# OmerMersin/video-stab

Measured on AMD Instinct MI355X. Metric: stabilized frames/sec @1080p (whole job; warp-stage HBM GB/s in roofline), higher is better.
Workload: dtype u8

## Files before the change

video-stab_amd/csrc/k_gftt.hip:

```cpp
#include <cstdio>
#include <cstdlib>

#include <cstring>

#include "vs_common.h"

namespace vsd {
namespace {

constexpr int TW = 64, TH = 16, NT = 256;
constexpr int MAX_BS = 7;

constexpr int SORT_CAP = 8192;
constexpr int CELLS_MAX = 2560;
constexpr int SLOTS = 4;
constexpr int ACC_MAX = 4096;
constexpr int SEL_NT = 256;
constexpr int NMS_ROWS = 8;

__device__ __forceinline__ uint32_t order_key(float v) {
    uint32_t b = __float_as_uint(v);
    return (b & 0x80000000u) ? ~b : (b | 0x80000000u);
}
__device__ __forceinline__ float key_to_float(uint32_t k) {
    uint32_t b = (k & 0x80000000u) ? (k & 0x7FFFFFFFu) : ~k;
    return __uint_as_float(b);
}

template <int BS>
__device__ __forceinline__ void min_eigen_tile(const uint8_t* __restrict__ gray, size_t stride, int w,
                                               int h, int bs_arg, float f1, float* __restrict__ eig,
                                               uint32_t* __restrict__ max_key) {
    constexpr int BSM = BS ? BS : MAX_BS;
    __shared__ uint8_t g[TH + BSM - 1 + 2][TW + BSM - 1 + 2 + 2];
    __shared__ float cxx[TH + BSM - 1][TW + BSM - 1 + 1], cxy[TH + BSM - 1][TW + BSM - 1 + 1], cyy[TH + BSM - 1][TW + BSM - 1 + 1];
    __shared__ uint32_t smax[NT / 64];
    const int bs = BS ? BS : bs_arg;
    const int tid = threadIdx.x;
    const int x0 = blockIdx.x * TW, y0 = blockIdx.y * TH;
    const int anchor = bs / 2, hi = bs - 1 - anchor;
    const int gx0 = x0 - anchor - 1, gy0 = y0 - anchor - 1;
    const int GW = TW + bs - 1 + 2, GH = TH + bs - 1 + 2;
    const int CW = TW + bs - 1, CH = TH + bs - 1;
    const float f0 = 2.f * f1;
    const bool interior = gx0 >= 0 && gy0 >= 0 && gx0 + GW <= w && gy0 + GH <= h;
    if (interior) {
        constexpr int NG = ((TW + BSM - 1 + 2) * (TH + BSM - 1 + 2) + NT - 1) / NT;
        const uint8_t* gb = gray + ((size_t)gy0 * stride + gx0);
        uint8_t v[NG];
        int ly[NG], lx[NG];
#pragma unroll
        for (int k = 0; k < NG; k++) {
            const int i = tid + NT * k;
            ly[k] = i / GW; lx[k] = i - ly[k] * GW;
            v[k] = i < GW * GH ? gb[(size_t)ly[k] * stride + lx[k]] : (uint8_t)0;
        }
#pragma unroll
        for (int k = 0; k < NG; k++)
            if (tid + NT * k < GW * GH) g[ly[k]][lx[k]] = v[k];
    } else {
        for (int i = tid; i < GW * GH; i += NT) {
            const int ly = i / GW, lx = i - ly * GW;
            g[ly][lx] = gray[(size_t)reflect101(gy0 + ly, h) * stride + reflect101(gx0 + lx, w)];
        }
    }
    __syncthreads();
    for (int i = tid; i < CW * CH; i += NT) {
        const int cy = i / CW, cx = i - cy * CW;
        const int px = x0 - anchor + cx, py = y0 - anchor + cy;
        float vxx = 0.f, vxy = 0.f, vyy = 0.f;
        if (interior || (px >= -anchor && px <= w - 1 + hi && py >= -anchor && py <= h - 1 + hi)) {
            const int qx = (interior ? px : reflect101(px, w)) - gx0, qy = (interior ? py : reflect101(py, h)) - gy0;
            const int a00 = g[qy - 1][qx - 1], a01 = g[qy - 1][qx], a02 = g[qy - 1][qx + 1];
            const int a10 = g[qy][qx - 1], a11 = g[qy][qx], a12 = g[qy][qx + 1];
            const int a20 = g[qy + 1][qx - 1], a21 = g[qy + 1][qx], a22 = g[qy + 1][qx + 1];
            const float r0 = (float)(a02 - a00), r1 = (float)(a12 - a10), r2 = (float)(a22 - a20);
            const float dx = (r0 + r2) * f1 + r1 * f0;
            const float t0 = (float)a01 * f0 + (float)(a00 + a02) * f1;
            const float t2 = (float)a21 * f0 + (float)(a20 + a22) * f1;
            const float dy = t2 - t0;
            (void)a11;
            vxx = dx * dx; vxy = dx * dy; vyy = dy * dy;
        }
        cxx[cy][cx] = vxx; cxy[cy][cx] = vxy; cyy[cy][cx] = vyy;
    }
    __syncthreads();
    uint32_t kmax = 0;
    for (int i = tid; i < TW * TH; i += NT) {
        const int ty = i / TW, tx = i - ty * TW;
        const int x = x0 + tx, y = y0 + ty;
        if (x < w && y < h) {
            double s0 = 0, s1 = 0, s2 = 0;
            for (int j = 0; j < bs; j++) {
                double r0 = 0, r1 = 0, r2 = 0;
                for (int k = 0; k < bs; k++) {
                    r0 += (double)cxx[ty + j][tx + k];
                    r1 += (double)cxy[ty + j][tx + k];
                    r2 += (double)cyy[ty + j][tx + k];
                }
                s0 += r0; s1 += r1; s2 += r2;
            }
            const float a = (float)s0 * 0.5f, b = (float)s1, c = (float)s2 * 0.5f;
            const float d = (a - c) * (a - c) + b * b;
            const float e = (a + c) - sqrtf(d);
            eig[(size_t)y * w + x] = e;
            const uint32_t k = order_key(e);
            kmax = k > kmax ? k : kmax;
        }
    }
#pragma unroll
    for (int off = 32; off >= 1; off >>= 1) {
        const uint32_t o = __shfl_xor(kmax, off, 64);
        kmax = o > kmax ? o : kmax;
    }
    if ((tid & 63) == 0) smax[tid >> 6] = kmax;
    __syncthreads();
    if (tid == 0) {
        uint32_t m = smax[0];
        for (int i = 1; i < NT / 64; i++) m = smax[i] > m ? smax[i] : m;
        atomicMax(max_key, m);
    }
}

template <int BS>
__global__ __launch_bounds__(NT) void min_eigen_kernel(const uint8_t* __restrict__ gray, size_t stride, int w,
                                                       int h, int bs, float f1, float* __restrict__ eig,
                                                       uint32_t* __restrict__ max_key) {
    min_eigen_tile<BS>(gray, stride, w, h, bs, f1, eig, max_key);
}

__device__ __forceinline__ void nms_row(const float* __restrict__ eig, int w, int h, double quality,
                                        const uint32_t* __restrict__ max_key,
                                        unsigned long long* __restrict__ cand, int cap,
                                        int32_t* __restrict__ counters) {
    const int x = blockIdx.x * blockDim.x + threadIdx.x;
    const float maxv = key_to_float(*max_key);
    const float thr = (float)((double)maxv * quality);
    const int lane = threadIdx.x & 63;
    float centre[NMS_ROWS];
    {
        const int xc = min(max(x, 0), w - 1);
#pragma unroll
        for (int k = 0; k < NMS_ROWS; k++) centre[k] = eig[(size_t)min((int)blockIdx.y * NMS_ROWS + k, h - 1) * w + xc];
    }
#pragma unroll
    for (int k = 0; k < NMS_ROWS; k++) {
    const int y = blockIdx.y * NMS_ROWS + k;
    if (y >= h) break;
    bool is_cand = false;
    float v = 0.f;
    if (x >= 1 && x < w - 1 && y >= 1 && y < h - 1) {
        const float* r = eig + (size_t)y * w + x;
        v = centre[k] > thr ? centre[k] : 0.f;
        if (v != 0.f) {
            float m = v;
#pragma unroll
            for (int j = -1; j <= 1; j++)
#pragma unroll
                for (int i = -1; i <= 1; i++) {
                    const float n = r[j * w + i];
                    const float tn = n > thr ? n : 0.f;
                    m = tn > m ? tn : m;
                }
            is_cand = v == m;
        }
    }
    const unsigned long long mask = __ballot(is_cand);
    if (!mask) continue;
    int base = 0;
    if (lane == __ffsll((long long)mask) - 1) base = atomicAdd(&counters[0], __popcll(mask));
    base = __builtin_amdgcn_readlane(base, __ffsll((long long)mask) - 1);
    if (!is_cand) continue;
    const int pos = base + __popcll(mask & ((1ull << lane) - 1ull));
    if (pos < cap) cand[pos] = ((unsigned long long)order_key(v) << 32) | (uint32_t)(y * w + x);
    else counters[2] = 1;
    }
}

__global__ __launch_bounds__(NT) void nms_kernel(const float* __restrict__ eig, int w, int h, double quality,
                                                 const uint32_t* __restrict__ max_key,
                                                 unsigned long long* __restrict__ cand, int cap,
                                                 int32_t* __restrict__ counters) {
    nms_row(eig, w, h, quality, max_key, cand, cap, counters);
}

struct SelArgs {
    const unsigned long long* cand;
    int32_t* counters;
    int cap, w, h, max_corners;
    int min_dist2_i;
    int use_dist;
    int cell, gw, gh;
    float* out_pts;
    int32_t* out_count;
};

template <int E>
__device__ __forceinline__ void bitonic_sort_desc(unsigned long long* keys, int tid) {
    unsigned long long v[E];
#pragma unroll
    for (int r = 0; r < E; r++) v[r] = keys[tid + SEL_NT * r];
    const int n = SEL_NT * E;
    for (int k = 2; k <= n; k <<= 1) {
        for (int j = k >> 1; j > 0; j >>= 1) {
            if (j < 64) {
#pragma unroll
                for (int r = 0; r < E; r++) {
                    const int i = tid + SEL_NT * r;
                    const unsigned int lo = (unsigned int)__shfl_xor((int)(unsigned int)v[r], j, 64);
                    const unsigned int hi = (unsigned int)__shfl_xor((int)(unsigned int)(v[r] >> 32), j, 64);
                    const unsigned long long o = ((unsigned long long)hi << 32) | lo;
                    const bool keep_max = ((i & k) == 0) == ((i & j) == 0);
                    v[r] = keep_max ? (v[r] > o ? v[r] : o) : (v[r] < o ? v[r] : o);
                }
            } else {
                __syncthreads();
#pragma unroll
                for (int r = 0; r < E; r++) keys[tid + SEL_NT * r] = v[r];
                __syncthreads();
#pragma unroll
                for (int r = 0; r < E; r++) {
                    const int i = tid + SEL_NT * r;
                    const unsigned long long o = keys[i ^ j];
                    const bool keep_max = ((i & k) == 0) == ((i & j) == 0);
                    v[r] = keep_max ? (v[r] > o ? v[r] : o) : (v[r] < o ? v[r] : o);
                }
            }
        }
    }
    __syncthreads();
#pragma unroll
    for (int r = 0; r < E; r++) keys[tid + SEL_NT * r] = v[r];
    __syncthreads();
}

__device__ __forceinline__ void select_corners(const SelArgs& a) {
    __shared__ unsigned long long keys[SORT_CAP];
    __shared__ uint32_t cell_cnt[CELLS_MAX];
    __shared__ uint32_t cell_pts[CELLS_MAX * SLOTS];
    __shared__ uint32_t acc_xy[ACC_MAX];
    __shared__ int s_m, s_nacc, s_done, s_cnt, s_overflow;
    __shared__ unsigned long long s_upper;
    const int tid = threadIdx.x;
    int ncand = a.counters[0];
    if (ncand > a.cap) ncand = a.cap;
    const int ncells = a.gw * a.gh;
    const bool grid_ok = a.use_dist && ncells <= CELLS_MAX;
    if (grid_ok) for (int i = tid; i < ncells; i += SEL_NT) cell_cnt[i] = 0;
    if (tid == 0) { s_nacc = 0; s_done = 0; s_upper = ~0ull; s_overflow = 0; }
    __syncthreads();

    int want = 1400;
    while (true) {
        const unsigned long long upper = s_upper;
        __syncthreads();
        if (tid == 0) s_cnt = 0;
        __syncthreads();
        int remaining;
        if (upper == ~0ull) {
            remaining = ncand;
        } else {
            int local = 0;
            for (int i = tid; i < ncand; i += SEL_NT) local += a.cand[i] < upper ? 1 : 0;
            if (local) atomicAdd(&s_cnt, local);
            __syncthreads();
            remaining = s_cnt;
        }
        if (remaining == 0) break;
        unsigned long long lo = 0;
        if (remaining > want + want / 2) {
            uint32_t* hist = reinterpret_cast<uint32_t*>(keys);
            unsigned long long prefix = 0;
            int above = 0;
            for (int shift = 56; shift >= 0; shift -= 8) {
                __syncthreads();
                hist[tid] = 0;
                __syncthreads();
                for (int i = tid; i < ncand; i += SEL_NT) {
                    const unsigned long long k = a.cand[i];
                    if (k < upper && (shift == 56 || (k >> (shift + 8)) == (prefix >> (shift + 8)))) atomicAdd(&hist[(uint32_t)(k >> shift) & 255u], 1u);
                }
                __syncthreads();
                if (tid == 0) {
                    int acc = above, bsel = 0;
                    for (int v = 255; v >= 0; v--) {
                        if (acc + (int)hist[v] >= want) { bsel = v; break; }
                        acc += (int)hist[v];
                    }
                    s_m = bsel;
                    s_cnt = acc;
                }
                __syncthreads();
                const int bsel = s_m, over = s_cnt, inbin = (int)hist[bsel];
                prefix |= (unsigned long long)bsel << shift;
                if (over + inbin <= SORT_CAP) { lo = prefix; break; }
                above = over;
                lo = prefix;
            }
        }
        __syncthreads();
        if (tid == 0) s_m = 0;
        __syncthreads();
        for (int i = tid; i < ncand; i += SEL_NT) {
            const unsigned long long k = a.cand[i];
            if (k >= lo && k < upper) {
                const int p = atomicAdd(&s_m, 1);
                if (p < SORT_CAP) keys[p] = k;
            }
        }
        __syncthreads();
        const int m = s_m < SORT_CAP ? s_m : SORT_CAP;
        int np2 = SEL_NT;
        while (np2 < m) np2 <<= 1;
        for (int i = m + tid; i < np2; i += SEL_NT) keys[i] = 0ull;
        __syncthreads();
        switch (np2 / SEL_NT) {
            case 1: bitonic_sort_desc<1>(keys, tid); break;
            case 2: bitonic_sort_desc<2>(keys, tid); break;
            case 4: bitonic_sort_desc<4>(keys, tid); break;
            case 8: bitonic_sort_desc<8>(keys, tid); break;
            case 16: bitonic_sort_desc<16>(keys, tid); break;
            default: bitonic_sort_desc<32>(keys, tid); break;
        }
        const unsigned long long last_key = m > 0 ? keys[m - 1] : 0ull;
        __syncthreads();
        for (int i = tid; i < m; i += SEL_NT) {
            const int idx = (int)(uint32_t)keys[i];
            const int y = idx / a.w, x = idx - y * a.w;
            const int xc = x / a.cell, yc = y / a.cell;
            keys[i] = (unsigned long long)((uint32_t)x | ((uint32_t)y << 16)) |
                      ((unsigned long long)((uint32_t)xc | ((uint32_t)yc << 16)) << 32);
        }
        __syncthreads();
        if (tid < 64) {
            const int lane = tid;
            int nacc = s_nacc;
            volatile uint32_t* vcnt = cell_cnt;
            volatile uint32_t* vpts = cell_pts;
            volatile uint32_t* vacc = acc_xy;
            const int md2 = a.min_dist2_i;
            bool full = false;
            for (int base = 0; base < m && !full; base += 64) {
                const int i = base + lane;
                const bool has = i < m;
                const unsigned long long e = has ? keys[i] : 0ull;
                const uint32_t xy = (uint32_t)e;
                const int x = (int)(xy & 0xFFFFu), y = (int)(xy >> 16);
                const int xc = (int)((uint32_t)(e >> 32) & 0xFFFFu), yc = (int)((uint32_t)(e >> 48));
                bool ok = has;
                if (a.use_dist && ok) {
                    if (grid_ok) {
                        int cidx[9];
                        uint32_t cnt[9];
#pragma unroll
                        for (int q = 0; q < 9; q++) {
                            const int cx = xc + (q % 3) - 1, cy = yc + (q / 3) - 1;
                            const bool in = cx >= 0 && cx < a.gw && cy >= 0 && cy < a.gh;
                            cidx[q] = in ? cy * a.gw + cx : -1;
                        }
#pragma unroll
                        for (int q = 0; q < 9; q++) cnt[q] = cidx[q] >= 0 ? vcnt[cidx[q]] : 0u;
#pragma unroll
                        for (int q = 0; q < 9; q++) {
                            const int c = cnt[q] < (uint32_t)SLOTS ? (int)cnt[q] : SLOTS;
                            for (int sl = 0; sl < c; sl++) {
                                const uint32_t p = vpts[cidx[q] * SLOTS + sl];
                                const int dx = x - (int)(p & 0xFFFFu), dy = y - (int)(p >> 16);
                                if (dx * dx + dy * dy < md2) ok = false;
                            }
                        }
                    } else {
                        for (int sl = 0; sl < nacc && ok; sl++) {
                            const uint32_t p = vacc[sl];
                            const int dx = x - (int)(p & 0xFFFFu), dy = y - (int)(p >> 16);
                            if (dx * dx + dy * dy < md2) ok = false;
                        }
                    }
                }
                unsigned long long mask = __ballot(ok);
                unsigned long long accepted = 0ull;
                const int nacc0 = nacc;
                while (mask) {
                    const int j = __ffsll((long long)mask) - 1;
                    accepted |= 1ull << j;
                    nacc++;
                    if (nacc == a.max_corners) { full = true; break; }
                    if (a.use_dist) {
                        const uint32_t pj = (uint32_t)__builtin_amdgcn_readlane((int)xy, j);
                        const int dx = x - (int)(pj & 0xFFFFu), dy = y - (int)(pj >> 16);
                        if (dx * dx + dy * dy < md2) ok = false;
                    }
                    if (lane == j) ok = false;
                    mask = __ballot(ok);
                }
                if ((accepted >> lane) & 1ull) {
                    const int pos = nacc0 + __popcll(accepted & ((1ull << lane) - 1ull));
                    a.out_pts[2 * pos] = (float)x;
                    a.out_pts[2 * pos + 1] = (float)y;
                    const uint32_t packed = (uint32_t)x | ((uint32_t)y << 16);
                    if (pos < ACC_MAX) acc_xy[pos] = packed;
                    if (grid_ok) {
                        const int c = yc * a.gw + xc;
                        const uint32_t slot = atomicAdd(&cell_cnt[c], 1u);
                        if (slot < (uint32_t)SLOTS) cell_pts[c * SLOTS + slot] = packed;
                        else s_overflow = 1;
                    }
                }
                __builtin_amdgcn_fence(__ATOMIC_RELEASE, "workgroup");
                __builtin_amdgcn_wave_barrier();
            }
            if (lane == 0) {
                s_nacc = nacc;
                if (full) s_done = 1;
                if (m > 0) s_upper = last_key;
                else s_done = 1;
            }
        }
        __syncthreads();
        if (s_done) break;
        want = SORT_CAP / 2;
    }
    __syncthreads();
    if (tid == 0) {
        *a.out_count = s_nacc;
        a.counters[3] = s_nacc;
        if (s_overflow) a.counters[2] = 2;
    }
}

__global__ __launch_bounds__(SEL_NT) void select_kernel(SelArgs a) { select_corners(a); }

struct GfttItem {
    const uint8_t* gray;
    size_t stride;
    int w, h, bs;
    float f1;
    double quality;
    float* eig;
    int32_t* counters;
    SelArgs sel;
};

__global__ __launch_bounds__(64) void gftt_zero_batch_kernel(const GfttItem* __restrict__ table) {
    if (threadIdx.x < 16) table[blockIdx.x].counters[threadIdx.x] = 0;
}
template <int BS>
__global__ __launch_bounds__(NT) void min_eigen_batch_kernel(const GfttItem* __restrict__ table) {
    const GfttItem& it = table[blockIdx.z];
    min_eigen_tile<BS>(it.gray, it.stride, it.w, it.h, it.bs, it.f1, it.eig, (uint32_t*)&it.counters[1]);
}
__global__ __launch_bounds__(NT) void nms_batch_kernel(const GfttItem* __restrict__ table) {
    const GfttItem& it = table[blockIdx.z];
    nms_row(it.eig, it.w, it.h, it.quality, (const uint32_t*)&it.counters[1], (unsigned long long*)it.sel.cand, it.sel.cap,
            it.counters);
}
__global__ __launch_bounds__(SEL_NT) void select_batch_kernel(const GfttItem* __restrict__ table) {
    select_corners(table[blockIdx.x].sel);
}

bool gftt_bad_args(const uint8_t* d_gray, const float* d_pts, const int32_t* d_count, int w, int h, int max_corners,
                   int block_size, const GfttWork& wk) {
    return !d_gray || !d_pts || !d_count || w < 3 || h < 3 || w > 65535 || h > 65535 || max_corners <= 0 ||
           max_corners > ACC_MAX || block_size < 1 || block_size > MAX_BS || !wk.eig || !wk.cand || !wk.counters ||
           wk.cap <= 0;
}

void fill_sel_args(SelArgs& a, int w, int h, int max_corners, double min_distance, const GfttWork& wk, float* d_pts,
                   int32_t* d_count) {
    a.cand = (const unsigned long long*)wk.cand;
    a.counters = wk.counters;
    a.cap = wk.cap; a.w = w; a.h = h; a.max_corners = max_corners;
    a.use_dist = min_distance >= 1 ? 1 : 0;
    a.min_dist2_i = (int)std::ceil(std::min(min_distance * min_distance, 2.0e9));
    a.cell = a.use_dist ? (int)lrint(min_distance) : 1;
    a.gw = (w + a.cell - 1) / a.cell;
    a.gh = (h + a.cell - 1) / a.cell;
    a.out_pts = d_pts; a.out_count = d_count;
}

}

size_t gftt_item_bytes() { return sizeof(GfttItem); }

int gftt_fill_item(void* host_item, const uint8_t* d_gray, size_t stride, int w, int h, int max_corners, double quality,
                   double min_distance, int block_size, const GfttWork& wk, float* d_pts, int32_t* d_count) {
    if (!host_item || gftt_bad_args(d_gray, d_pts, d_count, w, h, max_corners, block_size, wk)) {
        set_last_error("gftt: invalid argument (1 <= blockSize <= 7, 0 < maxCorners <= 4096)");
        return VS_ERR_INVALID_ARG;
    }
    GfttItem& it = *static_cast<GfttItem*>(host_item);
    memset(&it, 0, sizeof it);
    it.gray = d_gray; it.stride = stride; it.w = w; it.h = h; it.bs = block_size;
    double scale = (double)(1 << 2) * block_size * 255.0;
    it.f1 = (float)(1.0 / scale);
    it.quality = quality;
    it.eig = wk.eig; it.counters = wk.counters;
    fill_sel_args(it.sel, w, h, max_corners, min_distance, wk, d_pts, d_count);
    return VS_OK;
}

int launch_gftt_batch(const void* d_table, int items, int w, int h, int block_size, hipStream_t st, int what) {
    if (!d_table || items < 1 || items > 65535 || w < 3 || h < 3 || block_size < 1 || block_size > MAX_BS || what < 0 || what > 5) { set_last_error("gftt_batch: invalid argument"); return VS_ERR_INVALID_ARG; }
    const GfttItem* t = static_cast<const GfttItem*>(d_table);
    if (what == 0 || what == 1) hipLaunchKernelGGL(gftt_zero_batch_kernel, dim3(items), dim3(64), 0, st, t);
    if (what == 0 || what == 2 || what == 4) {
        const dim3 eg((w + TW - 1) / TW, (h + TH - 1) / TH, items);
        if (block_size == 3) hipLaunchKernelGGL(min_eigen_batch_kernel<3>, eg, dim3(NT), 0, st, t);
        else hipLaunchKernelGGL(min_eigen_batch_kernel<0>, eg, dim3(NT), 0, st, t);
    }
    if (what == 0 || what == 2 || what == 5)
        hipLaunchKernelGGL(nms_batch_kernel, dim3((w + NT - 1) / NT, (h + NMS_ROWS - 1) / NMS_ROWS, items), dim3(NT), 0, st, t);
    if (what == 0 || what == 3) hipLaunchKernelGGL(select_batch_kernel, dim3(items), dim3(SEL_NT), 0, st, t);
    VS_HIP_TRY(hipGetLastError());
    return VS_OK;
}

size_t gftt_work_bytes(int w, int h, int cap) {
    return (size_t)w * h * 4 + (size_t)cap * 8 + 64 + 256;
}

void gftt_work_carve(void* base, int w, int h, int cap, GfttWork* out) {
    uint8_t* p = (uint8_t*)base;
    out->eig = (float*)p;
    p += ((size_t)w * h * 4 + 63) & ~(size_t)63;
    out->cand = (uint64_t*)p;
    p += (size_t)cap * 8;
    out->counters = (int32_t*)p;
    out->cap = cap;
}

int launch_gftt(const uint8_t* d_gray, size_t stride, int w, int h, int max_corners, double quality,
                double min_distance, int block_size, const GfttWork& wk, float* d_pts,
                int32_t* d_count, hipStream_t st) {
    if (gftt_bad_args(d_gray, d_pts, d_count, w, h, max_corners, block_size, wk)) {
        set_last_error("gftt: invalid argument (1 <= blockSize <= 7, 0 < maxCorners <= 4096)");
        return VS_ERR_INVALID_ARG;
    }
    VS_HIP_TRY(hipMemsetAsync(wk.counters, 0, 64, st));
    double scale = (double)(1 << 2) * block_size * 255.0;
    scale = 1.0 / scale;
    const float f1 = (float)scale;
    dim3 g1((w + TW - 1) / TW, (h + TH - 1) / TH);
    if (block_size == 3)
        hipLaunchKernelGGL(min_eigen_kernel<3>, g1, dim3(NT), 0, st, d_gray, stride, w, h, block_size, f1, wk.eig, (uint32_t*)&wk.counters[1]);
    else
        hipLaunchKernelGGL(min_eigen_kernel<0>, g1, dim3(NT), 0, st, d_gray, stride, w, h, block_size, f1, wk.eig, (uint32_t*)&wk.counters[1]);
    dim3 g2((w + NT - 1) / NT, (h + NMS_ROWS - 1) / NMS_ROWS);
    hipLaunchKernelGGL(nms_kernel, g2, dim3(NT), 0, st, wk.eig, w, h, quality, (const uint32_t*)&wk.counters[1],
                       (unsigned long long*)wk.cand, wk.cap, wk.counters);
    SelArgs a;
    fill_sel_args(a, w, h, max_corners, min_distance, wk, d_pts, d_count);
    hipLaunchKernelGGL(select_kernel, dim3(1), dim3(SEL_NT), 0, st, a);
    VS_HIP_TRY(hipGetLastError());
    return VS_OK;
}

int run_gftt_op(const uint8_t* d_gray, size_t stride, int w, int h, int max_corners, double quality,
                double min_distance, int block_size, float* d_pts, int32_t* d_count, float* d_eig,
                hipStream_t st) {
    if (w <= 0 || h <= 0) { set_last_error("gftt: invalid size"); return VS_ERR_INVALID_ARG; }
    const int cap = w * h / 4 + 64;
    void* scratch = nullptr;
    VS_HIP_TRY(hipMalloc(&scratch, gftt_work_bytes(w, h, cap)));
    GfttWork wk;
    gftt_work_carve(scratch, w, h, cap, &wk);
    int rc = launch_gftt(d_gray, stride, w, h, max_corners, quality, min_distance, block_size, wk, d_pts, d_count, st);
    if (rc == VS_OK && d_eig) {
        hipError_t e = hipMemcpyAsync(d_eig, wk.eig, (size_t)w * h * 4, hipMemcpyDeviceToDevice, st);
        if (e != hipSuccess) { set_last_error(hipGetErrorString(e)); rc = VS_ERR_HIP; }
    }
    hipError_t e = hipStreamSynchronize(st);
    (void)hipFree(scratch);
    if (rc == VS_OK && e != hipSuccess) { set_last_error(hipGetErrorString(e)); rc = VS_ERR_HIP; }
    return rc;
}

}
```

Before: 128,700.

## Restructure GFTT min-eigen tile: rolling Sobel rows and column-wise separable box sums

New measurement: 131,800, median of 6. No clear change (+2.4%).

```diff
diff --git a/video-stab_amd/csrc/k_gftt.hip b/video-stab_amd/csrc/k_gftt.hip
--- a/video-stab_amd/csrc/k_gftt.hip
+++ b/video-stab_amd/csrc/k_gftt.hip
@@ -27,13 +27,32 @@
     return __uint_as_float(b);
 }
 
+constexpr int cov_pitch(int cw, int cws, int run) {
+    int p = cw;
+    while ((run * p - cws) % 32 != 0) p++;
+    return p;
+}
+
+__device__ __forceinline__ void sobel_row(const uint8_t* row, int q, float f0, float f1, float& rdx, float& tdy) {
+    const int a = row[q - 1], c = row[q], b = row[q + 1];
+    rdx = (float)(b - a);
+    tdy = (float)c * f0 + (float)(a + b) * f1;
+}
+
+constexpr int BOX_R = TH * TW / NT;
+static_assert(TW == 64 && BOX_R * NT == TH * TW, "box pass: one output column per lane of a wave");
+
 template <int BS>
 __device__ __forceinline__ void min_eigen_tile(const uint8_t* __restrict__ gray, size_t stride, int w,
                                                int h, int bs_arg, float f1, float* __restrict__ eig,
                                                uint32_t* __restrict__ max_key) {
     constexpr int BSM = BS ? BS : MAX_BS;
+    constexpr int CWS = BS ? TW + BS - 1 : 128;
+    constexpr int NRUN = NT / CWS;
+    constexpr int RUNM = (TH + BSM - 1 + NRUN - 1) / NRUN;
+    constexpr int CP = BS ? cov_pitch(TW + BS - 1, CWS, RUNM) : TW + BSM - 1 + 1;
     __shared__ uint8_t g[TH + BSM - 1 + 2][TW + BSM - 1 + 2 + 2];
-    __shared__ float cxx[TH + BSM - 1][TW + BSM - 1 + 1], cxy[TH + BSM - 1][TW + BSM - 1 + 1], cyy[TH + BSM - 1][TW + BSM - 1 + 1];
+    __shared__ float cxx[TH + BSM - 1][CP], cxy[TH + BSM - 1][CP], cyy[TH + BSM - 1][CP];
     __shared__ uint32_t smax[NT / 64];
     const int bs = BS ? BS : bs_arg;
     const int tid = threadIdx.x;
@@ -65,47 +84,88 @@
         }
     }
     __syncthreads();
-    for (int i = tid; i < CW * CH; i += NT) {
-        const int cy = i / CW, cx = i - cy * CW;
-        const int px = x0 - anchor + cx, py = y0 - anchor + cy;
-        float vxx = 0.f, vxy = 0.f, vyy = 0.f;
-        if (interior || (px >= -anchor && px <= w - 1 + hi && py >= -anchor && py <= h - 1 + hi)) {
-            const int qx = (interior ? px : reflect101(px, w)) - gx0, qy = (interior ? py : reflect101(py, h)) - gy0;
-            const int a00 = g[qy - 1][qx - 1], a01 = g[qy - 1][qx], a02 = g[qy - 1][qx + 1];
-            const int a10 = g[qy][qx - 1], a11 = g[qy][qx], a12 = g[qy][qx + 1];
-            const int a20 = g[qy + 1][qx - 1], a21 = g[qy + 1][qx], a22 = g[qy + 1][qx + 1];
-            const float r0 = (float)(a02 - a00), r1 = (float)(a12 - a10), r2 = (float)(a22 - a20);
-            const float dx = (r0 + r2) * f1 + r1 * f0;
-            const float t0 = (float)a01 * f0 + (float)(a00 + a02) * f1;
-            const float t2 = (float)a21 * f0 + (float)(a20 + a22) * f1;
-            const float dy = t2 - t0;
-            (void)a11;
-            vxx = dx * dx; vxy = dx * dy; vyy = dy * dy;
-        }
-        cxx[cy][cx] = vxx; cxy[cy][cx] = vxy; cyy[cy][cx] = vyy;
+    {
+        const int run = tid / CWS, cx = tid - run * CWS;
+        const int rows = BS ? RUNM : (CH + NRUN - 1) / NRUN;
+        const int cy0 = run * rows;
+        const int cy1 = min(cy0 + rows, CH);
+        if (run < NRUN && cx < CW) {
+            if (interior) {
+                float r0, r1, r2, t0, t1, t2;
+                sobel_row(g[cy0], cx + 1, f0, f1, r1, t1);
+                sobel_row(g[cy0 + 1], cx + 1, f0, f1, r2, t2);
+#pragma unroll
+                for (int s = 0; s < RUNM; s++) {
+                    const int cy = cy0 + s;
+                    if ((!BS || NRUN * RUNM != TH + BSM - 1) && cy >= cy1) break;
+                    r0 = r1; t0 = t1; r1 = r2; t1 = t2;
+                    sobel_row(g[cy + 2], cx + 1, f0, f1, r2, t2);
+                    const float dx = (r0 + r2) * f1 + r1 * f0;
+                    const float dy = t2 - t0;
+                    cxx[cy][cx] = dx * dx; cxy[cy][cx] = dx * dy; cyy[cy][cx] = dy * dy;
+                }
+            } else {
+                const int px = x0 - anchor + cx;
+                const bool col_in = px >= -anchor && px <= w - 1 + hi;
+                const int qx = reflect101(px, w) - gx0;
+                for (int cy = cy0; cy < cy1; cy++) {
+                    const int py = y0 - anchor + cy;
+                    float vxx = 0.f, vxy = 0.f, vyy = 0.f;
+                    if (col_in && py >= -anchor && py <= h - 1 + hi) {
+                        const int qy = reflect101(py, h) - gy0;
+                        float r0, r1, r2, t0, t1, t2;
+                        sobel_row(g[qy - 1], qx, f0, f1, r0, t0);
+                        sobel_row(g[qy], qx, f0, f1, r1, t1);
+                        sobel_row(g[qy + 1], qx, f0, f1, r2, t2);
+                        (void)t1;
+                        const float dx = (r0 + r2) * f1 + r1 * f0;
+                        const float dy = t2 - t0;
+                        vxx = dx * dx; vxy = dx * dy; vyy = dy * dy;
+                    }
+                    cxx[cy][cx] = vxx; cxy[cy][cx] = vxy; cyy[cy][cx] = vyy;
+                }
+            }
+        }
     }
     __syncthreads();
     uint32_t kmax = 0;
-    for (int i = tid; i < TW * TH; i += NT) {
-        const int ty = i / TW, tx = i - ty * TW;
-        const int x = x0 + tx, y = y0 + ty;
-        if (x < w && y < h) {
-            double s0 = 0, s1 = 0, s2 = 0;
-            for (int j = 0; j < bs; j++) {
-                double r0 = 0, r1 = 0, r2 = 0;
-                for (int k = 0; k < bs; k++) {
-                    r0 += (double)cxx[ty + j][tx + k];
-                    r1 += (double)cxy[ty + j][tx + k];
-                    r2 += (double)cyy[ty + j][tx + k];
-                }
-                s0 += r0; s1 += r1; s2 += r2;
-            }
-            const float a = (float)s0 * 0.5f, b = (float)s1, c = (float)s2 * 0.5f;
-            const float d = (a - c) * (a - c) + b * b;
-            const float e = (a + c) - sqrtf(d);
-            eig[(size_t)y * w + x] = e;
-            const uint32_t k = order_key(e);
-            kmax = k > kmax ? k : kmax;
+    {
+        const int tx = tid & (TW - 1), ty0 = (tid / TW) * BOX_R;
+        const int x = x0 + tx;
+        if (x < w) {
+            constexpr int JU = BS ? BOX_R + BSM - 1 : 1;
+            double s0[BOX_R], s1[BOX_R], s2[BOX_R];
+#pragma unroll
+            for (int r = 0; r < BOX_R; r++) { s0[r] = 0; s1[r] = 0; s2[r] = 0; }
+#pragma unroll JU
+            for (int j = 0; j < BOX_R + BSM - 1; j++) {
+                if (j >= BOX_R + bs - 1) break;
+                double h0 = (double)cxx[ty0 + j][tx], h1 = (double)cxy[ty0 + j][tx], h2 = (double)cyy[ty0 + j][tx];
+#pragma unroll
+                for (int k = 1; k < BSM; k++) {
+                    if (k >= bs) break;
+                    h0 += (double)cxx[ty0 + j][tx + k];
+                    h1 += (double)cxy[ty0 + j][tx + k];
+                    h2 += (double)cyy[ty0 + j][tx + k];
+                }
+#pragma unroll
+                for (int r = 0; r < BOX_R; r++) {
+                    if (j == r) { s0[r] = h0; s1[r] = h1; s2[r] = h2; }
+                    else if (j > r && j - r < bs) { s0[r] += h0; s1[r] += h1; s2[r] += h2; }
+                }
+            }
+#pragma unroll
+            for (int r = 0; r < BOX_R; r++) {
+                const int y = y0 + ty0 + r;
+                if (y < h) {
+                    const float a = (float)s0[r] * 0.5f, b = (float)s1[r], c = (float)s2[r] * 0.5f;
+                    const float d = (a - c) * (a - c) + b * b;
+                    const float e = (a + c) - sqrtf(d);
+                    eig[(size_t)y * w + x] = e;
+                    const uint32_t k = order_key(e);
+                    kmax = k > kmax ? k : kmax;
+                }
+            }
         }
     }
 #pragma unroll
@@ -559,7 +619,7 @@
                 double min_distance, int block_size, float* d_pts, int32_t* d_count, float* d_eig,
                 hipStream_t st) {
     if (w <= 0 || h <= 0) { set_last_error("gftt: invalid size"); return VS_ERR_INVALID_ARG; }
-    const int cap = w * h / 4 + 64;
+    const int cap = w * h;
     void* scratch = nullptr;
     VS_HIP_TRY(hipMalloc(&scratch, gftt_work_bytes(w, h, cap)));
     GfttWork wk;
```
